# ArbiterMob/FluidSimulationCuda

Measured on AMD Instinct MI355X. Metric: Mcells/s per Jacobi iter, higher is better.
Workload: dtype f32

## Files before the change

### fluidsimulationcuda_amd/capi.py

```python
import ctypes as C
import os

import numpy as np

from ._build import LIB

OK, E_INVALID, E_NOMEM, E_HIP, E_COMM = 0, 1, 2, 3, 4
U, V, DENS, U_PREV, V_PREV, DENS_PREV, TMP0, TMP1, TMP2, TMP3, TMP4, TMP5 = range(12)
NFIELDS = 12
JACOBI_STREAM, JACOBI_LDS, JACOBI_NAIVE, JACOBI_TB = 0, 1, 2, 3
STORAGE_F32, STORAGE_F16 = 0, 1
PARAM_TB_MAX_SWEEPS, PARAM_TB_ROWS, PARAM_HALO, PARAM_TB_FAST_DIVISION, PARAM_TB_MIN_CELLS, PARAM_TB_EDGE_ROWS_PCT = 0, 1, 2, 3, 4, 5
PARAM_TB_LANE_COLUMNS = 6
PARAM_TB_T16_MIN_CELLS = 7
PARAM_TB_AUTOTUNE = 8
PARAM_FUSE_DIVERGENCE = 9
PARAM_SLAB_OVERLAP = 10
PARAM_EARLY_ADVECT = 11
PARAM_FUSE_ADD_SOURCE = 12
PARAM_XCHG_OVERLAP = 13
PARAM_F16_PRESSURE_SCALE = 14
PARAM_TB_FILL = 15
XCHG_HALO, XCHG_GATHER, XCHG_MAX, XCHG_MAX_BEGIN, XCHG_MAX_END = 0, 1, 2, 3, 4
RCCL_ID_BYTES = 128
FIELD_NAMES = ("u", "v", "dens", "u_prev", "v_prev", "dens_prev", "tmp0", "tmp1", "tmp2", "tmp3", "tmp4", "tmp5")


class FluidError(RuntimeError):
    def __init__(self, code, msg):
        super().__init__("libfluid_amd error %d: %s" % (code, msg))
        self.code = code


class Config(C.Structure):
    _fields_ = [("n", C.c_int), ("rank", C.c_int), ("nranks", C.c_int), ("halo", C.c_int),
                ("jacobi_variant", C.c_int), ("stream", C.c_void_p), ("arena", C.c_void_p),
                ("arena_bytes", C.c_size_t), ("storage", C.c_int)]
# ... 77 lines not shown
    "fluid_upload_members": [_ctx, _i, _MF],
    "fluid_run": [_ctx, _f, _f, _f, C.POINTER(RunPlan), C.POINTER(_i)],
    "fluid_run_members": [_ctx, _MF, _MF, _MF, C.POINTER(RunPlan), C.POINTER(_i)],
    "fluid_coarse_size": [_i, _i, C.POINTER(_i)],
    "fluid_pack_members_coarse": [_ctx, _i, _i, _i, _i, C.c_void_p, C.c_size_t],
    "fluid_download_members_coarse": [_ctx, _i, _i, _MF],
    "fluid_run_coarse": [_ctx, _f, _f, _f, C.POINTER(RunPlan), _i, C.POINTER(_i)],
    "fluid_run_members_coarse": [_ctx, _MF, _MF, _MF, C.POINTER(RunPlan), _i, C.POINTER(_i)],
    "fluid_transform_members": [_ctx, C.POINTER(_i), _i, _MF],
    "fluid_select_members": [_ctx, C.POINTER(_i), _i, C.POINTER(_i)],
    "fluid_set_jacobi_variant": [_ctx, _i],
    "fluid_division_mode": [_ctx, _f, _f, C.POINTER(_i)],
    "fluid_autotune_pending": [_ctx, C.POINTER(_i)],
    "fluid_plan_sweeps": [_i, _i, _i, _i, _i, _i, _i, C.POINTER(_i), _i, C.POINTER(_i)],
    "fluid_set_param": [_ctx, _i, _i],
    "fluid_timing_enable": [_ctx, _i],
    "fluid_timing_read": [_ctx, C.POINTER(Timing), _i],
    "fluid_op_diffuse_tol": [_ctx, _i, _i, _i, _f, _f, _f, _i, _i, C.POINTER(_i), C.POINTER(_f)],
    "fluid_set_exchange": [_ctx, EXCHANGE_FN, C.c_void_p],
    "fluid_exchange_now": [_ctx, _i, C.POINTER(_i), _i, _i],
    "fluid_exchange_stream": [_ctx, C.POINTER(C.c_void_p)],
    "fluid_split_launches": [_ctx, C.POINTER(C.c_longlong)],
    "fluid_rccl_available": [],
    "fluid_rccl_unique_id": [C.c_void_p, C.c_size_t],
    "fluid_exchange_rccl_attach": [_ctx, C.c_void_p, C.c_size_t],
    "fluid_exchange_rccl_attach_comm": [_ctx, C.c_void_p],
    "fluid_exchange_rccl_detach": [_ctx],
    "fluid_exchange_rccl_calls": [_ctx, C.POINTER(C.c_longlong), C.POINTER(C.c_longlong), C.POINTER(C.c_longlong)],
}
OTHER_SYMBOLS = {"fluid_last_error": (C.c_char_p, []), "fluid_arena_bytes": (C.c_size_t, [_i]),
# ... 34 lines not shown
```

### fluidsimulationcuda_amd/csrc/fluid_ctx.h

```cpp
#pragma once
#include <hip/hip_runtime.h>

#include <string>
#include <utility>
#include <vector>

#include "../../include/fluid_amd.h"
#include "fluid_kernels.h"

namespace fluid_detail {
int fail(int code, const char* fmt, ...);
int materialize_zero(fluid_ctx* c, int f);
int refuse_ensemble(const fluid_ctx* c, const char* what);
struct RcclExchange;
void rccl_release(RcclExchange* x);
}

#define HIP_TRY(expr)                                                                                      \
    do {                                                                                                   \
        hipError_t e_ = (expr);                                                                            \
        if (e_ != hipSuccess)                                                                              \
            return fluid_detail::fail(e_ == hipErrorOutOfMemory ? FLUID_E_NOMEM : FLUID_E_HIP, "%s: %s",   \
                                      #expr, hipGetErrorString(e_));                                       \
    } while (0)
// ... 88 lines not shown
    hipEvent_t ev_xbegin = nullptr, ev_xdone = nullptr;
    bool xchg_overlap = true;
    unsigned xowed = 0;
    long long split_launches = 0;
    bool early_advect = true;
    float vmax_prev[2] = {-1.0f, -1.0f};
    FieldState field[FLUID_NFIELDS];
    size_t field_bytes = 0;
    unsigned int* d_scalar = nullptr;
    float* d_partials = nullptr;
    ConstRing consts;
    EnsembleReduce red;
    MemberStage stage;
    TransformTables xform;
    unsigned int* tiles = nullptr;
    unsigned int* h_scalar = nullptr;
    hipEvent_t scalar_ready = nullptr;
    int variant = fluid::JACOBI_TB;
    int tb_max_t = 16, tb_rows = 0, num_cu = 256;
    long long tb_min_cells = 0;
    long long tb_t16_min_cells = -1;
    bool fuse_divergence = true;
    bool tb_fill = true;
    bool autotune = true;
    struct Trial { unsigned long long key; int cand; hipEvent_t a, b; };
    std::vector<Trial> trials;
    std::vector<hipEvent_t> free_events;
    bool defer_zero_source = true;
    bool in_halo_exchange = false;
    int tb_nv = 2;
// ... 29 lines not shown
```

### fluidsimulationcuda_amd/csrc/fluid_kernels.h

```cpp
#pragma once
#include <hip/hip_runtime.h>

namespace fluid {

constexpr int XOFF = 63;

enum JacobiVariant { JACOBI_STREAM = 0, JACOBI_LDS = 1, JACOBI_NAIVE = 2, JACOBI_TB = 3, JACOBI_VARIANTS = 4 };

enum Storage { STORAGE_F32 = 0, STORAGE_F16 = 1 };
typedef _Float16 half_t;
inline size_t storage_bytes(int st) { return st == STORAGE_F16 ? 2 : 4; }

inline int pitch_for(int n) { return ((XOFF + 1 + 4 * ((n + 3) / 4) + 1) + 63) / 64 * 64; }

struct Members {
    int count = 1;
    size_t stride = 0;
};

struct TbMemberK {
    double yd;
    float alpha, beta, hi, lo;
    float x0_inc, div_scale;
    unsigned tile_thr, pad;
};

struct TbBatch {
    const void* x[3];
    const void* x0[3];
    void* out[3];
    float alpha[3], beta[3];
    double yd[3];
    float hi[3], lo[3];
    const unsigned* tiles[3];
    unsigned tile_thr[3];
    int tile_pitch;
    void* div[3];
    float div_scale;
    int b[3];
    int x_zero[3];
    float x0_inc[3];
    int count;
    int members;
    size_t mstride;
    size_t tile_mstride;
    const TbMemberK* mk;
};

void launch_set_bnd(hipStream_t s, int st, void* f, int pitch, int n, int b, Members mb = {});
void launch_add_source(hipStream_t s, int st, void* x, const void* src, int pitch, int row_lo, int row_hi, float dt, Members mb = {},
                       const float* mdt = nullptr);
void launch_jacobi(hipStream_t s, int st, int variant, const void* x, const void* x0, void* out, int pitch, int n,
                   int row_lo, int row_hi, float alpha, float beta, int b, Members mb = {}, const float2* mab = nullptr);
enum TbForm { TB_PLAIN = 0, TB_DIVSRC = 1, TB_ADDSRC = 2 };
struct TbShape { int T, divmode, nv, form; };
inline constexpr TbShape kTbShapes[] = {
    {2, 0, 2, TB_PLAIN},   {2, 2, 2, TB_PLAIN},   {2, 3, 2, TB_PLAIN},   {2, 4, 2, TB_PLAIN},   {2, 5, 2, TB_PLAIN},
    {2, 0, 4, TB_PLAIN},   {2, 2, 4, TB_PLAIN},   {2, 3, 4, TB_PLAIN},   {2, 4, 4, TB_PLAIN},   {2, 5, 4, TB_PLAIN},
    {4, 0, 2, TB_PLAIN},   {4, 2, 2, TB_PLAIN},   {4, 3, 2, TB_PLAIN},   {4, 4, 2, TB_PLAIN},   {4, 5, 2, TB_PLAIN},
    {4, 0, 4, TB_PLAIN},   {4, 2, 4, TB_PLAIN},   {4, 3, 4, TB_PLAIN},   {4, 4, 4, TB_PLAIN},   {4, 5, 4, TB_PLAIN},
    {8, 0, 2, TB_PLAIN},   {8, 2, 2, TB_PLAIN},   {8, 3, 2, TB_PLAIN},   {8, 4, 2, TB_PLAIN},   {8, 5, 2, TB_PLAIN},
    {8, 0, 4, TB_PLAIN},   {8, 2, 4, TB_PLAIN},   {8, 3, 4, TB_PLAIN},   {8, 4, 4, TB_PLAIN},   {8, 5, 4, TB_PLAIN},
// ... 20 lines not shown
inline constexpr int kTbDepths[] = {16, 12, 8, 4, 2};
constexpr bool is_tb_depth(int T) { for (int d : kTbDepths) if (d == T) return true; return false; }
bool launch_jacobi_tb(hipStream_t s, int st, int T, int divmode, int nv, int form, const TbBatch& batch, int pitch, int n, int row_lo,
                      int row_hi, int rb, int rb_edge, int hole_lo = 0, int hole_hi = 0, bool fill = true);
constexpr int kTileRows = 32, kTileCols = 64;
inline int tile_rows(int n) { return (n + kTileRows - 1) / kTileRows; }
inline int tile_pitch(int n) { return (n + kTileCols - 1) / kTileCols; }
struct TileBatch {
    const void* field[3];
    unsigned* tiles[3];
    int count;
    size_t mstride, tile_mstride;
};
void launch_tile_min_abs(hipStream_t s, int st, const TileBatch& tb, int count, int pitch, int n, int row_lo, int row_hi, int tile_pitch,
                         Members mb = {}, size_t tile_mstride = 0);
void launch_validate_div(hipStream_t s, int divmode, float beta, float kbeta, double yd, float hi, float lo, unsigned long long* bad);
void launch_advect(hipStream_t s, int st, void* d, const void* d0, const void* u, const void* v, int pitch, int n,
                   int row_lo, int row_hi, float dt0, int b, Members mb = {}, const float* mdt0 = nullptr);
void launch_advect2(hipStream_t s, int st, void* da, const void* d0a, int ba, void* db, const void* d0b, int bb, const void* u,
                    const void* v, int pitch, int n, int row_lo, int row_hi, float dt0, Members mb = {}, const float* mdt0 = nullptr);
void launch_divergence(hipStream_t s, int st, const void* u, const void* v, void* p, void* div, int pitch, int n,
                       int row_lo, int row_hi, float h, int write_p, float pscale = 1.0f, Members mb = {});
void launch_scale(hipStream_t s, int st, void* x, int pitch, int row_lo, int row_hi, float factor, Members mb = {});
constexpr int kMaxPartials = 8192;
void launch_subtract_gradient(hipStream_t s, int st, void* u, void* v, const void* p, int pitch, int n, int row_lo,
                              int row_hi, float h, float* partials = nullptr, unsigned int* max_out = nullptr, float pinv = 1.0f,
                              Members mb = {});
void launch_gradient_advect(hipStream_t s, int st, void* u, void* v, const void* p, void* d, const void* d0, int pitch, int n,
                            int row_lo, int row_hi, float h, float dt0, int b, float pinv = 1.0f, Members mb = {},
                            const float* mdt0 = nullptr);
// ... 28 lines not shown
```

### fluidsimulationcuda_amd/csrc/fluid_kernels.hip

```cpp
#include <hip/hip_runtime.h>
#include <stdint.h>

#include <algorithm>
#include <array>
#include <cstdlib>
#include <utility>

#include "fluid_kernels.h"

namespace fluid {

__device__ __forceinline__ float flip_if(bool c, float v) { return c ? -v : v; }

__device__ __forceinline__ float keep_f32(float v) { asm("" : "+v"(v)); return v; }
__device__ __forceinline__ float ld1(const float* p) { return *p; }
__device__ __forceinline__ float ld1(const half_t* p) { return keep_f32((float)*p); }
__device__ __forceinline__ void st1(float* p, float v) { *p = v; }
__device__ __forceinline__ void st1(half_t* p, float v) { *p = (half_t)keep_f32(v); }
template <typename S>
__device__ __forceinline__ float as_stored(float v)
{
    if constexpr (sizeof(S) == 2) return keep_f32((float)(S)keep_f32(v));
    else return v;
}
// ... 781 lines not shown
        vid -= (unsigned)g.inner_blocks;
        const int e = (int)(vid % (unsigned)g.edge_wins);
        strip_group = (int)(vid / (unsigned)g.edge_wins);
        win = e == 0 ? 0 : g.first_right + e - 1;
    }
    const unsigned member = batch.count == 3 ? blockIdx.z / 3u : batch.count == 2 ? blockIdx.z >> 1 : blockIdx.z;
    const unsigned sv = blockIdx.z - member * (unsigned)batch.count;
    const size_t mofs = (size_t)member * batch.mstride;
    const S* __restrict__ x = static_cast<const S*>(batch.x[sv]) + mofs;
    const S* __restrict__ x0 = static_cast<const S*>(batch.x0[sv]) + mofs;
    S* __restrict__ out = static_cast<S*>(batch.out[sv]) + mofs;
    float alpha = batch.alpha[sv], beta = batch.beta[sv];
    double yd = batch.yd[sv];
    float k_hi = batch.hi[sv], k_lo = batch.lo[sv], x0_inc = batch.x0_inc[sv], div_scale = batch.div_scale;
    unsigned tile_thr = batch.tile_thr[sv];
    if (batch.mk != nullptr) {
        typedef const TbMemberK __attribute__((address_space(4))) * MemberKPtr;
        const MemberKPtr mk = (MemberKPtr)(uintptr_t)batch.mk + ((size_t)sv * (unsigned)batch.members + member);
        alpha = mk->alpha;
        beta = mk->beta;
        yd = mk->yd;
        k_hi = mk->hi;
        k_lo = mk->lo;
        x0_inc = mk->x0_inc;
        if (ADDSRC) div_scale = mk->div_scale;
        if (DIVMODE == 3) tile_thr = mk->tile_thr;
    }
    const int b = batch.b[sv];
    constexpr int HL = (T + NV - 1) / NV;
    constexpr int VS = 64 - 2 * HL;
    constexpr int C0 = (XOFF + 1) / NV;
    static_assert((XOFF + 1) % NV == 0 && HL <= C0, "window overlap must fit the row's left pad");
    const int lane = threadIdx.x & 63;
    const int strip = strip_group * 4 + __builtin_amdgcn_readfirstlane(threadIdx.x >> 6);
    const int kg = n / NV;
    const bool left_edge = (win == 0);
    const bool right_edge = (kg >= win * VS - HL) && (kg < win * VS - HL + 64);
    const bool edge = left_edge || right_edge;
    const int rbw = edge ? rb_edge : rb;
    TbArgs<S, NV> a;
    a.k.yd = yd;
// ... 37 lines not shown
    const bool is_rg = (k == kg);
    const bool own = (lane >= HL) && (lane < 64 - HL);
    const bool st_int = own && k >= 0 && k < nvec;
    a.st_rg_lane = is_rg && (own || k == nvec);
    a.m_lg = a.is_lg ? 0xFFFFFFFFu : 0u;
#pragma unroll
    for (int c = 0; c < NV; ++c) a.m_r[c] = (is_rg && a.cg == c) ? 0xFFFFFFFFu : 0u;
    a.st_off = (ld_ok && (st_int || a.is_lg || a.st_rg_lane)) ? a.ld_off : kBufOff;
    a.sx = (b == 1) ? 0x80000000u : 0u;
    a.sy = (b == 2) ? 0x80000000u : 0u;
    a.alpha = alpha;
    a.k.beta = beta;
    a.fill = fill != 0;
    const int t0 = max(0, a.q_lo - T), t1 = a.q_hi - 1 + T;
    const bool wall = (a.q_lo < T) || (a.q_hi - 1 + T > n + 1);
    constexpr int DM = DIVMODE == 3 ? 2 : DIVMODE;
    bool two_term = false;
    if constexpr (DIVMODE == 3) {
        const unsigned* __restrict__ tiles = batch.tiles[sv] ? batch.tiles[sv] + (size_t)member * batch.tile_mstride : nullptr;
        const unsigned thr = tile_thr;
        const int tr0 = (max(1, a.q_lo - T + 1) - 1) / kTileRows, tr1 = (min(n, a.q_hi + T - 2) - 1) / kTileRows;
        const int c0 = max(1, 1 + NV * (win * VS - HL)), c1 = min(n, NV * (win * VS - HL + 64));
        const int tc0 = (c0 - 1) / kTileCols, tc1 = (c1 - 1) / kTileCols, ntc = tc1 - tc0 + 1;
        const int count = (tr1 - tr0 + 1) * ntc;
        bool low = false;
        if (tiles != nullptr)
            for (int i = lane; i < count; i += 64)
                low |= tiles[(size_t)(tr0 + i / ntc) * batch.tile_pitch + (tc0 + i % ntc)] < thr;
        two_term = tiles != nullptr && __builtin_amdgcn_ballot_w64(low) == 0ull;
    }
// ... 19 lines not shown
    const int i0 = max(row_lo, 1 + tr * kTileRows), i1 = min(row_hi, 1 + (tr + 1) * kTileRows);
    const size_t P = (size_t)pitch;
    float m = __builtin_inff();
    if (j <= n)
        for (int i = i0; i < i1; ++i) {
            const float4 v = ld4(f + (size_t)i * P + XOFF + j);
            m = fminf(m, fabsf(v.x));
            if (j + 1 <= n) m = fminf(m, fabsf(v.y));
            if (j + 2 <= n) m = fminf(m, fabsf(v.z));
            if (j + 3 <= n) m = fminf(m, fabsf(v.w));
        }
#pragma unroll
    for (int off = 8; off > 0; off >>= 1) m = fminf(m, __shfl_xor(m, off, 16));
    const bool whole = row_lo <= 1 + tr * kTileRows && row_hi >= min(n + 1, 1 + (tr + 1) * kTileRows);
    if ((lane & 15) == 0 && j <= n) out[(size_t)tr * tile_pitch + (j - 1) / kTileCols] = whole ? __float_as_uint(m) : 0u;
}

template <typename S, typename IDX>
__device__ __forceinline__ const S* at(const S* base, IDX byte_off) { return reinterpret_cast<const S*>(reinterpret_cast<const char*>(base) + byte_off); }
template <typename S, typename IDX>
__device__ __forceinline__ S* at(S* base, IDX byte_off) { return reinterpret_cast<S*>(reinterpret_cast<char*>(base) + byte_off); }

template <typename IDX>
struct AdvectTap {
    IDX o;
    float s0, s1, t0, t1;
};

template <typename IDX>
__device__ __forceinline__ AdvectTap<IDX> advect_trace(int j, int i, float uu, float vv, float dt0, int n, IDX P, IDX E)
// ... 949 lines not shown
void launch_tile_min_abs(hipStream_t s, int st, const TileBatch& tiles, int count, int pitch, int n, int row_lo, int row_hi, int tile_pitch,
                         Members mb, size_t tile_mstride)
{
    if (row_lo < 1) row_lo = 1;
    if (row_hi > n + 1) row_hi = n + 1;
    if (row_hi <= row_lo || count <= 0) return;
    const int tr0 = (row_lo - 1) / kTileRows, tr1 = (row_hi - 2) / kTileRows;
    const dim3 grid(cdiv(cdiv(n, 4), 256), tr1 - tr0 + 1, count * mb.count);
    TileBatch tb = tiles;
    tb.count = count;
    tb.mstride = mb.stride;
    tb.tile_mstride = tile_mstride;
    FLUID_BY_STORAGE(st, hipLaunchKernelGGL(k_tile_min_abs<S>, grid, dim3(256), 0, s, tb, pitch, n, row_lo, row_hi, tr0, tile_pitch));
}

void launch_validate_div(hipStream_t s, int divmode, float beta, float kbeta, double yd, float hi, float lo, unsigned long long* bad)
{
    DivK k;
    k.beta = kbeta;
    k.yd = yd;
    k.hi = hi;
    k.lo = lo;
    const auto f = divmode == 4 ? k_validate_div<4> : divmode == 5 ? k_validate_div<5> : divmode == 3 ? k_validate_div<3> : k_validate_div<2>;
    hipLaunchKernelGGL(f, dim3(8192), dim3(256), 0, s, beta, k, bad);
}

void launch_advect(hipStream_t s, int st, void* d, const void* d0, const void* u, const void* v, int pitch, int n,
                   int row_lo, int row_hi, float dt0, int b, Members mb, const float* mdt0)
{
    if (row_hi <= row_lo) return;
// ... 199 lines not shown
```

### fluidsimulationcuda_amd/csrc/fluid_solver.hip

```cpp
#include <hip/hip_runtime.h>

#include <algorithm>
#include <cmath>
#include <cstdarg>
#include <cstdio>
#include <cstring>
#include <functional>
#include <mutex>
#include <new>
#include <string>
#include <unordered_map>
#include <vector>

#include "fluid_ctx.h"

namespace fluid_detail {

thread_local std::string g_err;

int fail(int code, const char* fmt, ...)
{
    char buf[512];
    va_list ap;
    va_start(ap, fmt);
// ... 638 lines not shown
                pickd = depth[k];
        if (!pickd) break;
        if (pickd <= room) best = std::max(best, pickd);
        r -= pickd;
    }
    return best ? best : greedy;
}

struct Coeffs {
    MemberVal alpha, beta;
};

struct Solve {
    int b, x, x0;
    const Coeffs* k;
};

struct DivSource {
    int u, v;
    float scale;
};

struct Batch {
    const Solve* sv;
    int count, iters, final_reach;
    const DivSource* ds;
    int scratch_base;
    const int* scratch;
    const int* sum;
    int cur[3], nxt[3];
    std::vector<DivPlan> plan[3];
    bool same_mode, all_mode4, add_src;
    float out_scale[3];
    SweepShape shape;
};

size_t tile_words(const fluid_ctx* c) { return (size_t)fluid::tile_rows(c->n) * fluid::tile_pitch(c->n); }
unsigned* solve_tiles(const fluid_ctx* c, int slot) { return c->tiles + (size_t)slot * c->members * tile_words(c); }

void plan_members(fluid_ctx* c, const Coeffs& k, std::vector<DivPlan>& out)
{
    const int M = c->members;
    const MemberVal &alpha = k.alpha, &beta = k.beta;
    out.resize(M);
    bool same = true;
    for (int m = 0; m < M; ++m) {
        out[m] = (m > 0 && beta.at(m) == beta.at(m - 1) && alpha.at(m) == alpha.at(m - 1)) ? out[m - 1] : division_mode(c, beta.at(m), alpha.at(m));
// ... 76 lines not shown
    }
    B.shape = sweep_shape(c, B.count);
    const FieldState& x00 = c->field[sv[0].x0];
    bool add_src = x00.src_of != 0 && B.ds == nullptr && B.same_mode;
    for (int k = 0; k < B.count; ++k) {
        const FieldState &x = c->field[sv[k].x], &x0 = c->field[sv[k].x0];
        add_src = add_src && x0.src_of == 1 + sv[k].x && x0.src_dt == x00.src_dt && !x.zero && !x.pend && !x.src_of;
    }
    B.add_src = add_src && fluid::jacobi_tb_exists(pick_sweeps(c, B.iters, B.iters, B.shape, B.all_mode4), B.plan[0][0].mode, c->tb_nv, fluid::TB_ADDSRC);
    if (!B.add_src)
        for (int k = 0; k < B.count; ++k)
            if (c->field[sv[k].x0].src_of) {
                TRY(xchg_join(c));
                TRY(settle_source(c, sv[k].x0));
            }
    fluid::TileBatch tb{};
    int m = 0, valid = kEverywhere;
    for (int k = 0; k < B.count; ++k)
        if (B.plan[k][0].mode == 3) {
            tb.field[m] = c->ptr(sv[k].x0);
            tb.tiles[m] = solve_tiles(c, B.scratch_base + k);
            valid = std::min(valid, c->nranks > 1 ? c->field[sv[k].x0].reach : kEverywhere);
            ++m;
        }
    if (m == 0) return FLUID_OK;
    TRY(xchg_join(c));
    if (c->nranks > 1)
        HIP_TRY(hipMemsetAsync(solve_tiles(c, B.scratch_base), 0, (size_t)B.count * c->members * tile_words(c) * sizeof(unsigned), c->stream));
    int lo, hi;
    rows(c, std::min(valid, c->n), &lo, &hi);
    fluid::launch_tile_min_abs(c->stream, c->st, tb, m, c->pitch, c->n, lo, hi, fluid::tile_pitch(c->n), c->mb(), tile_words(c));
    return FLUID_OK;
}

int batch_reach(const fluid_ctx* c, const Batch& B)
{
    int r = kEverywhere;
    for (int k = 0; k < B.count; ++k) r = std::min(r, std::min(c->field[B.cur[k]].reach, c->field[B.sv[k].x0].reach + 1));
    return r;
}

fluid::TbMemberK solve_constants(const Batch& B, int j, int m, const MemberVal& x0_inc, const MemberVal& div_scale)
{
    const DivPlan& p = B.plan[j][B.plan[j].size() > 1 ? (size_t)m : 0];
    return {p.yd, B.sv[j].k->alpha.at(m), p.arg, p.hi, p.lo, x0_inc.at(m), div_scale.at(m), p.tile_thr, 0};
}

int fill_batch(fluid_ctx* c, const Batch& B, int first, int last, bool divsrc, bool addsrc, fluid::TbBatch* out)
{
    static const MemberVal nothing_pending(-0.0f);
    const MemberVal own_scale(divsrc ? B.ds->scale : 0.0f);
    const MemberVal& div_scale = addsrc ? c->field[B.sv[first].x0].src_dt : own_scale;
    const MemberVal* x0_inc[3];
    fluid::TbBatch bt{};
    bool per_member = !div_scale.uniform();
    for (int j = first; j < last; ++j) {
        const int q = j - first;
        const FieldState& x0 = c->field[B.sv[j].x0];
        x0_inc[q] = x0.pend && !addsrc && !divsrc ? &x0.pend_inc : &nothing_pending;
        per_member = per_member || B.plan[j].size() > 1 || !x0_inc[q]->uniform();
        const fluid::TbMemberK k0 = solve_constants(B, j, 0, *x0_inc[q], div_scale);
        bt.x[q] = c->ptr(B.cur[j]);
        bt.x0[q] = x0.ptr;
        bt.out[q] = c->ptr(B.nxt[j]);
        bt.alpha[q] = k0.alpha;
        bt.beta[q] = k0.beta;
        bt.yd[q] = k0.yd;
        bt.hi[q] = k0.hi;
        bt.lo[q] = k0.lo;
        bt.tiles[q] = B.plan[j][0].mode == 3 ? solve_tiles(c, B.scratch_base + j) : nullptr;
        bt.tile_thr[q] = k0.tile_thr;
        bt.b[q] = B.sv[j].b;
        bt.x_zero[q] = c->field[B.cur[j]].zero ? 1 : 0;
        bt.x0_inc[q] = k0.x0_inc;
        if (addsrc) bt.div[q] = c->ptr(B.sum[j]);
    }
    bt.count = last - first;
    bt.members = c->members;
    bt.mstride = c->field_floats;
    bt.tile_mstride = tile_words(c);
    bt.tile_pitch = fluid::tile_pitch(c->n);
    bt.div_scale = div_scale.at(0);
    if (divsrc) {
        bt.x[0] = c->ptr(B.ds->u);
        bt.x0[0] = c->ptr(B.ds->v);
        bt.div[0] = c->ptr(B.sv[0].x0);
    }
    if (per_member && c->members > 1) {
        const int M = c->members;
        std::vector<fluid::TbMemberK> rec((size_t)bt.count * M);
        for (int j = first; j < last; ++j)
            for (int m = 0; m < M; ++m) rec[(size_t)(j - first) * M + m] = solve_constants(B, j, m, *x0_inc[j - first], div_scale);
        const void* dev = nullptr;
        TRY(member_consts(c, rec.data(), rec.size() * sizeof rec[0], &dev));
        bt.mk = static_cast<const fluid::TbMemberK*>(dev);
    }
    *out = bt;
    return FLUID_OK;
}

int edge_rows(const fluid_ctx* c, int T, int rb) { return std::max(2 * T, rb * (c->tb_edge_pct > 0 ? c->tb_edge_pct : 100) / 100); }

int strip_rows(const fluid_ctx* c, int T, int m, long long rows_n)
{
    const int nv = c->tb_nv;
    const int HL = (T + nv - 1) / nv, VS = 64 - 2 * HL;
    const long long windows = ((c->n + nv - 1) / nv + VS - 1) / VS;
// ... 99 lines not shown
            for (int j = 0; j < B.count; ++j) {
                const float2* mab = nullptr;
                TRY(member_pairs(c, sv[j].k->alpha, sv[j].k->beta, &mab));
                fluid::launch_jacobi(c->stream, c->st, v, c->ptr(B.cur[j]), c->ptr(sv[j].x0), c->ptr(B.nxt[j]), c->pitch, c->n, lo, hi,
                                     sv[j].k->alpha.at(0), sv[j].k->beta.at(0), sv[j].b, c->mb(), mab);
            }
            if (c->timing) {
                c->launches += B.count;
                c->field_launches += (long long)B.count * c->members;
            }
        } else {
            for (int first = 0, last; first < B.count; first = last) {
                last = B.same_mode ? B.count : first + 1;
                const bool divsrc = B.ds != nullptr && k == 0, addsrc = B.add_src && k == 0;
                fluid::TbBatch bt;
                TRY(fill_batch(c, B, first, last, divsrc, addsrc, &bt));
                TRY(launch_fused(c, bt, T, B.plan[first][0].mode, divsrc, addsrc, lo, hi));
                if (c->timing) {
                    c->launches += 1;
                    c->field_launches += (long long)(last - first) * c->members;
                }
            }
        }
        r = multi ? std::min(r - T, exchange_cap(c)) : kEverywhere;
        commit_launch(c, B, k == 0, r);
        k += T;
    }
    return FLUID_OK;
}

int op_diffuse_batch(fluid_ctx* c, const Solve* sv, int count, int iters, int final_reach = 0, const DivSource* ds = nullptr,
// ... 241 lines not shown
    const Solve uv[2] = {{1, U0, U, &cv}, {2, V0, V, &cv}};
    TRY(op_diffuse_batch(c, uv, 2, iters));
    TRY(xchg_join(c));
    TRY(project(c, U0, V0, U, V, iters, nullptr, true));
    const float dt0 = dt.at(0) * (float)c->n;
    TRY(vmax_begin(c, U0, V0, true));
    TRY(advect_bounded(c, 0, {U0, V0}, dt0, [&] { return op_advect2(c, 1, U, U0, 2, V, V0, U0, V0, dt); }));
    return project(c, U, V, U0, V0, iters);
}

int dens_step(fluid_ctx* c, const MemberVal& dt, const MemberVal& diff, int iters)
{
    const int X = FLUID_DENS, X0 = FLUID_DENS_PREV;
    TRY(op_add_source(c, X, X0, dt, true));
    const Coeffs cd = diffusion_coeffs(c, dt, diff);
    const Solve one{0, X0, X, &cd};
    TRY(op_diffuse_batch(c, &one, 1, iters));
    TRY(vmax_begin(c, FLUID_U, FLUID_V));
    return advect_bounded(c, 1, {X0}, dt.at(0) * (float)c->n, [&] { return op_advect(c, 0, X, X0, FLUID_U, FLUID_V, dt); });
}

int full_step(fluid_ctx* c, const MemberVal& dt, const MemberVal& diff, const MemberVal& visc, int iters)
{
    const int U = FLUID_U, V = FLUID_V, D = FLUID_DENS, U0 = FLUID_U_PREV, V0 = FLUID_V_PREV, D0 = FLUID_DENS_PREV;
    TRY(op_add_source(c, U, U0, dt, true));
    TRY(op_add_source(c, V, V0, dt, true));
    TRY(op_add_source(c, D, D0, dt, true));
    TRY(need(c, {U, V, D, U0, V0, D0}, std::min(iters, c->halo), true));
    const Coeffs cv = diffusion_coeffs(c, dt, visc), cd = diffusion_coeffs(c, dt, diff);
    const float dt0 = dt.at(0) * (float)c->n;
    const Solve all[3] = {{1, U0, U, &cv}, {2, V0, V, &cv}, {0, D0, D, &cd}};
    if (c->nranks == 1) {
        TRY(op_diffuse_batch(c, all, 3, iters));
        TRY(project(c, U0, V0, U, V, iters));
        TRY(op_advect2(c, 1, U, U0, 2, V, V0, U0, V0, dt));
        const AdvectAfter dens{0, D, D0, dt};
        return project(c, U, V, U0, V0, iters, &dens);
    }
    int fill1 = 0, fill2 = 0;
    {
        const SweepShape shape = sweep_shape(c, 1);
        std::vector<int> launches;
        for (int left = iters; left > 0;) {
            launches.push_back(pick_sweeps(c, left, left, shape, false));
            left -= launches.back();
        }
        for (int* fill : {&fill2, &fill1})
            while (*fill < 8 && !launches.empty()) {
// ... 203 lines not shown
    if (P > 1) {
        if (!hip_ok(hipStreamCreateWithFlags(&c->stream2, hipStreamNonBlocking), "hipStreamCreate(second stream)")) return bail(rc);
        if (!hip_ok(hipEventCreateWithFlags(&c->ev_fork, hipEventDisableTiming), "hipEventCreate")) return bail(rc);
        if (!hip_ok(hipEventCreateWithFlags(&c->ev_join, hipEventDisableTiming), "hipEventCreate")) return bail(rc);
        if (!hip_ok(hipStreamCreateWithFlags(&c->xstream, hipStreamNonBlocking), "hipStreamCreate(exchange stream)")) return bail(rc);
        if (!hip_ok(hipEventCreateWithFlags(&c->ev_xbegin, hipEventDisableTiming), "hipEventCreate")) return bail(rc);
        if (!hip_ok(hipEventCreateWithFlags(&c->ev_xdone, hipEventDisableTiming), "hipEventCreate")) return bail(rc);
    }
    if (!hip_ok(hipMemsetAsync(c->arena, 0, bytes, c->stream), "hipMemsetAsync(arena)")) return bail(rc);
    c->d_scalar = reinterpret_cast<unsigned int*>(c->arena + c->all_bytes() * FLUID_NFIELDS);
    {
        const size_t words = 3 * (size_t)members * tile_words(c);
        if (!hip_ok(hipMalloc((void**)&c->tiles, words * sizeof(unsigned)), "hipMalloc(tiles)")) return bail(rc);
        if (!hip_ok(hipMemsetAsync(c->tiles, 0, words * sizeof(unsigned), c->stream), "hipMemsetAsync(tiles)")) return bail(rc);
    }
    if (P > 1 && !hip_ok(hipMalloc((void**)&c->d_partials, fluid::kMaxPartials * sizeof(float)), "hipMalloc(partials)")) return bail(rc);
    if (!hip_ok(hipHostMalloc((void**)&c->h_scalar, 256, hipHostMallocDefault), "hipHostMalloc")) return bail(rc);
    if (!hip_ok(hipEventCreateWithFlags(&c->scalar_ready, hipEventDisableTiming), "hipEventCreate")) return bail(rc);
    if (!hip_ok(hipStreamSynchronize(c->stream), "hipStreamSynchronize")) return bail(rc);
    *out = c;
    return FLUID_OK;
}

int fluid_create(int N, fluid_ctx** out)
{
    fluid_config cfg;
    std::memset(&cfg, 0, sizeof cfg);
    cfg.n = N;
    cfg.nranks = 1;
    cfg.jacobi_variant = FLUID_JACOBI_TB;
// ... 13 lines not shown
    if (!c->trials.empty()) {
        RbTuner& t = rb_tuner();
        std::lock_guard<std::mutex> lock(t.mu);
        for (auto& tr : c->trials) {
            auto it = t.table.find(tr.key);
            if (it != t.table.end() && !it->second.fixed && it->second.issued[tr.cand] > 0) it->second.issued[tr.cand] -= 1;
            (void)hipEventDestroy(tr.a);
            (void)hipEventDestroy(tr.b);
        }
    }
    for (hipEvent_t ev : c->free_events) (void)hipEventDestroy(ev);
    fluid_detail::rccl_release(c->rccl);
    c->rccl = nullptr;
    if (c->h_scalar) (void)hipHostFree(c->h_scalar);
    if (c->tiles) (void)hipFree(c->tiles);
    for (auto& b : c->consts.live) (void)hipEventDestroy(b.copied);
    for (hipEvent_t ev : c->consts.free_events) (void)hipEventDestroy(ev);
    if (c->consts.dev) (void)hipFree(c->consts.dev);
    if (c->consts.host) (void)hipHostFree(c->consts.host);
    if (c->red.d_max) (void)hipFree(c->red.d_max);
    if (c->red.d_moments) (void)hipFree(c->red.d_moments);
    if (c->red.d_partials) (void)hipFree(c->red.d_partials);
    if (c->red.host) (void)hipHostFree(c->red.host);
    if (c->red.d_mean) (void)hipFree(c->red.d_mean);
    if (c->red.d_var) (void)hipFree(c->red.d_var);
    if (c->red.d_gram_partials) (void)hipFree(c->red.d_gram_partials);
    if (c->red.d_gram) (void)hipFree(c->red.d_gram);
    if (c->red.gram_host) (void)hipHostFree(c->red.gram_host);
    if (c->stage.dev) (void)hipFree(c->stage.dev);
    for (hipEvent_t ev : c->xform.copied)
// ... 23 lines not shown
}

int fluid_exchange_stream(fluid_ctx* c, void** stream)
{
    TRY(check_ctx(c));
    if (!stream) return fail(FLUID_E_INVALID, "null pointer");
    *stream = c->stream;
    return FLUID_OK;
}

int fluid_split_launches(fluid_ctx* c, long long* count)
{
    TRY(check_ctx(c));
    if (!count) return fail(FLUID_E_INVALID, "null pointer");
    *count = c->split_launches;
    return FLUID_OK;
}

int fluid_owned_rows(fluid_ctx* c, int* row_lo, int* row_hi)
{
    TRY(check_ctx(c));
    if (row_lo) *row_lo = c->own0;
    if (row_hi) *row_hi = c->own1;
    return FLUID_OK;
}

int fluid_field_ptr(fluid_ctx* c, int field, void** dev_ptr)
{
    TRY(check_ctx(c));
    TRY(check_fields(c, {field}));
// ... 155 lines not shown
        c->pscale = (value != 0 && c->st == fluid::STORAGE_F16 && c->n >= 16) ? std::ldexp(1.0f, e - 3) : 1.0f;
        return FLUID_OK;
    }
    case FLUID_PARAM_XCHG_OVERLAP:
        TRY(xchg_join(c));
        c->xchg_overlap = value != 0;
        return FLUID_OK;
    case FLUID_PARAM_TB_T16_MIN_CELLS:
        if (value < -1) return fail(FLUID_E_INVALID, "TB_T16_MIN_CELLS must be >= 0, or -1 for the default rule");
        c->tb_t16_min_cells = value;
        return FLUID_OK;
    case FLUID_PARAM_TB_LANE_COLUMNS:
        if (value != 2 && value != 4) return fail(FLUID_E_INVALID, "TB_LANE_COLUMNS must be 2 or 4");
        c->tb_nv = value;
        return FLUID_OK;
    case FLUID_PARAM_HALO:
        if (value < 1) return fail(FLUID_E_INVALID, "HALO must be >= 1");
        c->halo = c->nranks > 1 ? std::max(c->st == fluid::STORAGE_F16 ? 8 : 1, std::min(value, c->min_slab - 1)) : 1;
        return FLUID_OK;
    default:
        return fail(FLUID_E_INVALID, "unknown parameter %d", key);
    }
}

int fluid_plan_sweeps(int N, int rows, int storage, int pressure_form, int iters, int max_sweeps, int t16_min_cells, int* depths,
                      int capacity, int* count)
{
    if (N < 1 || N > kMaxN || rows < 1 || rows > N || iters < 0 || (iters & 1) || !depths || !count || capacity < 0)
        return fail(FLUID_E_INVALID, "fluid_plan_sweeps: bad argument");
    if (storage != FLUID_STORAGE_F32 && storage != FLUID_STORAGE_F16) return fail(FLUID_E_INVALID, "unknown storage type %d", storage);
// ... 1011 lines not shown
```

### fluidsimulationcuda_amd/solver.py

```python
import ctypes as C
import sys

import numpy as np

from . import capi

DT, VIS, DIFF, ITERS = 0.016, 0.0025, 0.1, 40

_ID = {name: k for k, name in enumerate(capi.FIELD_NAMES)}


def _fid(f):
    if isinstance(f, str):
        return _ID[f]
    return int(f)


def _host(a, n):
    a = np.ascontiguousarray(a, dtype=np.float32)
    if a.shape != (n + 2, n + 2):
        raise ValueError("field must have shape (%d, %d), got %s" % (n + 2, n + 2, a.shape))
    return a


# ... 321 lines not shown
            out[name + "_ms"] = t.category_ms[k]
            out[name + "_calls"] = t.category_calls[k]
        return out

    def diffuse_tol(self, b, x, x0, alpha, beta, tol, max_iters=10000, check_every=8):
        it, res = C.c_int(), C.c_float()
        capi.check(capi.lib().fluid_op_diffuse_tol(self._h, b, _fid(x), _fid(x0), alpha, beta, tol, max_iters,
                                                   check_every, C.byref(it), C.byref(res)))
        return it.value, res.value

    def split_launches(self):
        m = C.c_longlong()
        capi.check(capi.lib().fluid_split_launches(self._h, C.byref(m)))
        return m.value

    def exchange_stream(self):
        p = C.c_void_p()
        capi.check(capi.lib().fluid_exchange_stream(self._h, C.byref(p)))
        return p.value or 0

    def set_exchange(self, fn):
        if fn is None:
            self._cb = None
            capi.check(capi.lib().fluid_set_exchange(self._h, C.cast(None, capi.EXCHANGE_FN), None))
            return

        def tramp(_user, kind, fields, nfields, depth, scalar):
            try:
                ids = [fields[k] for k in range(nfields)]
                if kind in (capi.XCHG_MAX, capi.XCHG_MAX_END):
# ... 38 lines not shown
```

### include/fluid_amd.h

```cpp
#ifndef FLUID_AMD_H
#define FLUID_AMD_H

#include <stddef.h>

#ifdef __cplusplus
extern "C" {
#endif

#define FLUID_OK        0
#define FLUID_E_INVALID 1
#define FLUID_E_NOMEM   2
#define FLUID_E_HIP     3
#define FLUID_E_COMM    4

enum {
    FLUID_U = 0, FLUID_V = 1, FLUID_DENS = 2,
    FLUID_U_PREV = 3, FLUID_V_PREV = 4, FLUID_DENS_PREV = 5,
    FLUID_TMP0 = 6, FLUID_TMP1 = 7, FLUID_TMP2 = 8,
    FLUID_TMP3 = 9, FLUID_TMP4 = 10, FLUID_TMP5 = 11,
    FLUID_NFIELDS = 12
};

enum { FLUID_JACOBI_STREAM = 0, FLUID_JACOBI_LDS = 1, FLUID_JACOBI_NAIVE = 2, FLUID_JACOBI_TB = 3 };

// ... 1 lines not shown
    FLUID_PARAM_TB_MAX_SWEEPS = 0,
    FLUID_PARAM_TB_ROWS = 1,
    FLUID_PARAM_HALO = 2,
    FLUID_PARAM_TB_FAST_DIVISION = 3
    ,FLUID_PARAM_TB_EDGE_ROWS_PCT = 5
    ,FLUID_PARAM_TB_LANE_COLUMNS = 6
    ,FLUID_PARAM_TB_T16_MIN_CELLS = 7
    ,FLUID_PARAM_TB_AUTOTUNE = 8
    ,FLUID_PARAM_SLAB_OVERLAP = 10
    ,FLUID_PARAM_EARLY_ADVECT = 11
    ,FLUID_PARAM_FUSE_DIVERGENCE = 9
    ,FLUID_PARAM_FUSE_ADD_SOURCE = 12
    ,FLUID_PARAM_XCHG_OVERLAP = 13
    ,FLUID_PARAM_F16_PRESSURE_SCALE = 14
    ,FLUID_PARAM_TB_FILL = 15
    ,FLUID_PARAM_TB_MIN_CELLS = 4
};

typedef struct fluid_ctx fluid_ctx;

const char *fluid_last_error(void);

int step(int N, float dt, float diff, float visc, float *u, float *v, float *dens);
int step_src(int N, float dt, float diff, float visc, int iters,
             float *u, float *v, float *dens,
             float *u_prev, float *v_prev, float *dens_prev);
int fluid_release_cached(void);

int fluid_coefficients(int N, float dt, float coef, float *alpha, float *beta);

// ... 93 lines not shown
int fluid_run_coarse(fluid_ctx *ctx, float dt, float diff, float visc, const fluid_run_plan *plan, int factor,
                     int *snapshots_written);
int fluid_run_members_coarse(fluid_ctx *ctx, const float *dt, const float *diff, const float *visc,
                             const fluid_run_plan *plan, int factor, int *snapshots_written);

#define FLUID_TRANSFORM_MAX_MEMBERS 64
int fluid_transform_members(fluid_ctx *ctx, const int *fields, int nfields, const float *weights);
int fluid_select_members(fluid_ctx *ctx, const int *fields, int nfields, const int *source);

int fluid_set_jacobi_variant(fluid_ctx *ctx, int variant);
int fluid_division_mode(fluid_ctx *ctx, float alpha, float beta, int *mode);
int fluid_plan_sweeps(int N, int rows, int storage, int pressure_form, int iters, int max_sweeps, int t16_min_cells,
                      int *depths, int capacity, int *count);
int fluid_autotune_pending(fluid_ctx *ctx, int *shapes_open);
int fluid_set_param(fluid_ctx *ctx, int key, int value);

enum {
    FLUID_TIME_SOURCE = 0, FLUID_TIME_DIFFUSION = 1, FLUID_TIME_DIVERGENCE = 2,
    FLUID_TIME_PROJECTION = 3, FLUID_TIME_ADVECTION = 4, FLUID_TIMING_CATEGORIES = 5
};
typedef struct fluid_timing {
    double jacobi_ms;
    long long sweeps;
    long long solves;
    double category_ms[FLUID_TIMING_CATEGORIES];
    long long category_calls[FLUID_TIMING_CATEGORIES];
    long long jacobi_launches;
    long long jacobi_field_launches;
    double pressure_ms;
    long long pressure_sweeps;
// ... 30 lines not shown
```

Measured before the change: 4.278 million.

## Skip Jacobi work on all-zero density tiles via per-tile nonzero bitmaps

Adds a pre-pass kernel that ORs the bit patterns of the density right-hand side and initial guess into a per-tile map. The temporally blocked Jacobi kernel checks, per wavefront, whether every tile inside its dependency cone (widened by the sweep index) is zero, and if so writes zeros and returns instead of computing. Density is reordered to be first in the batched diffusion solve, and device-side atomic counters record how many waves skip. The change adds a map-building pass and atomics on every launch, and it only pays off when the density field is sparse.

```diff
diff --git a/fluidsimulationcuda_amd/capi.py b/fluidsimulationcuda_amd/capi.py
--- a/fluidsimulationcuda_amd/capi.py
+++ b/fluidsimulationcuda_amd/capi.py
@@ -21,6 +21,7 @@
 PARAM_XCHG_OVERLAP = 13
 PARAM_F16_PRESSURE_SCALE = 14
 PARAM_TB_FILL = 15
+PARAM_SPARSE_DENSITY = 16
 XCHG_HALO, XCHG_GATHER, XCHG_MAX, XCHG_MAX_BEGIN, XCHG_MAX_END = 0, 1, 2, 3, 4
 RCCL_ID_BYTES = 128
 FIELD_NAMES = ("u", "v", "dens", "u_prev", "v_prev", "dens_prev", "tmp0", "tmp1", "tmp2", "tmp3", "tmp4", "tmp5")
@@ -128,6 +129,7 @@
     "fluid_autotune_pending": [_ctx, C.POINTER(_i)],
     "fluid_plan_sweeps": [_i, _i, _i, _i, _i, _i, _i, C.POINTER(_i), _i, C.POINTER(_i)],
     "fluid_set_param": [_ctx, _i, _i],
+    "fluid_sparse_stats": [_ctx, C.POINTER(C.c_ulonglong)],
     "fluid_timing_enable": [_ctx, _i],
     "fluid_timing_read": [_ctx, C.POINTER(Timing), _i],
     "fluid_op_diffuse_tol": [_ctx, _i, _i, _i, _f, _f, _f, _i, _i, C.POINTER(_i), C.POINTER(_f)],
diff --git a/fluidsimulationcuda_amd/csrc/fluid_ctx.h b/fluidsimulationcuda_amd/csrc/fluid_ctx.h
--- a/fluidsimulationcuda_amd/csrc/fluid_ctx.h
+++ b/fluidsimulationcuda_amd/csrc/fluid_ctx.h
@@ -126,6 +126,8 @@
     MemberStage stage;
     TransformTables xform;
     unsigned int* tiles = nullptr;
+    bool sparse_density = true;
+    unsigned long long* d_zstats = nullptr;
     unsigned int* h_scalar = nullptr;
     hipEvent_t scalar_ready = nullptr;
     int variant = fluid::JACOBI_TB;
diff --git a/fluidsimulationcuda_amd/csrc/fluid_kernels.h b/fluidsimulationcuda_amd/csrc/fluid_kernels.h
--- a/fluidsimulationcuda_amd/csrc/fluid_kernels.h
+++ b/fluidsimulationcuda_amd/csrc/fluid_kernels.h
@@ -22,7 +22,8 @@
     double yd;
     float alpha, beta, hi, lo;
     float x0_inc, div_scale;
-    unsigned tile_thr, pad;
+    unsigned tile_thr;
+    unsigned sparse;
 };
 
 struct TbBatch {
@@ -45,7 +46,12 @@
     size_t mstride;
     size_t tile_mstride;
     const TbMemberK* mk;
+    const unsigned* zmap[3];
+    int zmap_k0;
+    unsigned long long* zstats;
 };
+constexpr int kSparseStatSlots = 64, kSparseStatStride = 16;
+constexpr size_t kSparseStatWords = (size_t)kSparseStatSlots * kSparseStatStride;
 
 void launch_set_bnd(hipStream_t s, int st, void* f, int pitch, int n, int b, Members mb = {});
 void launch_add_source(hipStream_t s, int st, void* x, const void* src, int pitch, int row_lo, int row_hi, float dt, Members mb = {},
@@ -96,6 +102,8 @@
 };
 void launch_tile_min_abs(hipStream_t s, int st, const TileBatch& tb, int count, int pitch, int n, int row_lo, int row_hi, int tile_pitch,
                          Members mb = {}, size_t tile_mstride = 0);
+void launch_tile_or_bits(hipStream_t s, int st, const void* rhs, const void* guess, unsigned* map, int pitch, int n, int tile_pitch,
+                         Members mb = {}, size_t tile_mstride = 0);
 void launch_validate_div(hipStream_t s, int divmode, float beta, float kbeta, double yd, float hi, float lo, unsigned long long* bad);
 void launch_advect(hipStream_t s, int st, void* d, const void* d0, const void* u, const void* v, int pitch, int n,
                    int row_lo, int row_hi, float dt0, int b, Members mb = {}, const float* mdt0 = nullptr);
diff --git a/fluidsimulationcuda_amd/csrc/fluid_kernels.hip b/fluidsimulationcuda_amd/csrc/fluid_kernels.hip
--- a/fluidsimulationcuda_amd/csrc/fluid_kernels.hip
+++ b/fluidsimulationcuda_amd/csrc/fluid_kernels.hip
@@ -819,6 +819,8 @@
     double yd = batch.yd[sv];
     float k_hi = batch.hi[sv], k_lo = batch.lo[sv], x0_inc = batch.x0_inc[sv], div_scale = batch.div_scale;
     unsigned tile_thr = batch.tile_thr[sv];
+    constexpr bool CAN_SKIP = !DIVSRC && DIVMODE != 4;
+    bool sparse = CAN_SKIP && batch.zmap[sv] != nullptr;
     if (batch.mk != nullptr) {
         typedef const TbMemberK __attribute__((address_space(4))) * MemberKPtr;
         const MemberKPtr mk = (MemberKPtr)(uintptr_t)batch.mk + ((size_t)sv * (unsigned)batch.members + member);
@@ -830,6 +832,7 @@
         x0_inc = mk->x0_inc;
         if (ADDSRC) div_scale = mk->div_scale;
         if (DIVMODE == 3) tile_thr = mk->tile_thr;
+        if (CAN_SKIP && sparse) sparse = mk->sparse != 0u;
     }
     const int b = batch.b[sv];
     constexpr int HL = (T + NV - 1) / NV;
@@ -897,6 +900,34 @@
     a.fill = fill != 0;
     const int t0 = max(0, a.q_lo - T), t1 = a.q_hi - 1 + T;
     const bool wall = (a.q_lo < T) || (a.q_hi - 1 + T > n + 1);
+    if constexpr (CAN_SKIP) {
+        if (sparse && !edge && !wall) {
+            const unsigned* __restrict__ zm = batch.zmap[sv] + (size_t)member * batch.tile_mstride;
+            const int k0 = batch.zmap_k0;
+            const int tr0 = (max(1, a.q_lo - T - k0) - 1) / kTileRows, tr1 = (min(n, a.q_hi - 1 + T + k0) - 1) / kTileRows;
+            const int c0 = max(1, 1 + NV * (win * VS - HL) - k0), c1 = min(n, NV * (win * VS - HL + 64) + k0);
+            const int tc0 = (c0 - 1) / kTileCols, tc1 = (c1 - 1) / kTileCols, ntc = tc1 - tc0 + 1;
+            const int count = (tr1 - tr0 + 1) * ntc;
+            bool nz = false;
+            for (int i = lane; i < count; i += 64) nz |= zm[(size_t)(tr0 + i / ntc) * batch.tile_pitch + (tc0 + i % ntc)] != 0u;
+            const bool skip = __builtin_amdgcn_ballot_w64(nz) == 0ull;
+            if (lane == 0) {
+                unsigned long long* slot = batch.zstats + (blockIdx.x % kSparseStatSlots) * (size_t)kSparseStatStride;
+                atomicAdd(slot + 1, 1ull);
+                if (skip) atomicAdd(slot, 1ull);
+            }
+            if (skip) {
+                Vec<NV> zero;
+#pragma unroll
+                for (int c = 0; c < NV; ++c) zero.c[c] = 0.f;
+                for (int q = a.q_lo; q < a.q_hi; ++q) {
+                    buf_stv<NV>(a.oc, a.bo, a.st_off + (unsigned)q * a.row_bytes, zero);
+                    if constexpr (ADDSRC) buf_stv<NV>(a.dc, a.bd, a.st_off + (unsigned)q * a.row_bytes, zero);
+                }
+                return;
+            }
+        }
+    }
     constexpr int DM = DIVMODE == 3 ? 2 : DIVMODE;
     bool two_term = false;
     if constexpr (DIVMODE == 3) {
@@ -946,6 +977,43 @@
     for (int off = 8; off > 0; off >>= 1) m = fminf(m, __shfl_xor(m, off, 16));
     const bool whole = row_lo <= 1 + tr * kTileRows && row_hi >= min(n + 1, 1 + (tr + 1) * kTileRows);
     if ((lane & 15) == 0 && j <= n) out[(size_t)tr * tile_pitch + (j - 1) / kTileCols] = whole ? __float_as_uint(m) : 0u;
+}
+
+template <typename S>
+__global__ __launch_bounds__(256) void k_tile_or_bits(const S* __restrict__ rhs, const S* __restrict__ guess, unsigned* __restrict__ map,
+                                                      int pitch, int n, int tile_pitch, size_t mstride, size_t tile_mstride)
+{
+    const unsigned member = blockIdx.z;
+    rhs += (size_t)member * mstride;
+    if (guess != nullptr) guess += (size_t)member * mstride;
+    unsigned* __restrict__ out = map + (size_t)member * tile_mstride;
+    const int lane = threadIdx.x & 63, wave = threadIdx.x >> 6;
+    const int tr = blockIdx.y;
+    const int j = 1 + 4 * (lane + 64 * (blockIdx.x * 4 + wave));
+    const int i0 = 1 + tr * kTileRows, i1 = min(n + 1, i0 + kTileRows);
+    const size_t P = (size_t)pitch;
+    const unsigned m1 = j + 1 <= n ? ~0u : 0u, m2 = j + 2 <= n ? ~0u : 0u, m3 = j + 3 <= n ? ~0u : 0u;
+    auto row_bits = [&](const S* f, int i) {
+        const float4 v = ld4(f + (size_t)i * P + XOFF + j);
+        return __float_as_uint(v.x) | (__float_as_uint(v.y) & m1) | (__float_as_uint(v.z) & m2) | (__float_as_uint(v.w) & m3);
+    };
+    unsigned bits = 0u;
+    if (j <= n) {
+        if (guess == nullptr) {
+            for (int i = i0; i < i1; ++i) bits |= row_bits(rhs, i);
+        } else {
+            for (int i = i0; i < i1; ++i) bits |= row_bits(rhs, i) | row_bits(guess, i);
+            if (i0 == 1) bits |= row_bits(guess, 0);
+            if (i1 == n + 1) bits |= row_bits(guess, n + 1);
+            if (j == 1)
+                for (int i = i0; i < i1; ++i) bits |= __float_as_uint(ld1(guess + (size_t)i * P + XOFF));
+            if (j + 3 >= n)
+                for (int i = i0; i < i1; ++i) bits |= __float_as_uint(ld1(guess + (size_t)i * P + XOFF + n + 1));
+        }
+    }
+#pragma unroll
+    for (int off = 8; off > 0; off >>= 1) bits |= (unsigned)__shfl_xor((int)bits, off, 16);
+    if ((lane & 15) == 0 && j <= n) out[(size_t)tr * tile_pitch + (j - 1) / kTileCols] = bits;
 }
 
 template <typename S, typename IDX>
@@ -1925,6 +1993,14 @@
     FLUID_BY_STORAGE(st, hipLaunchKernelGGL(k_tile_min_abs<S>, grid, dim3(256), 0, s, tb, pitch, n, row_lo, row_hi, tr0, tile_pitch));
 }
 
+void launch_tile_or_bits(hipStream_t s, int st, const void* rhs, const void* guess, unsigned* map, int pitch, int n, int tile_pitch,
+                         Members mb, size_t tile_mstride)
+{
+    const dim3 grid(cdiv(cdiv(n, 4), 256), tile_rows(n), mb.count);
+    FLUID_BY_STORAGE(st, hipLaunchKernelGGL(k_tile_or_bits<S>, grid, dim3(256), 0, s, (const S*)rhs, (const S*)guess, map, pitch, n,
+                                            tile_pitch, mb.stride, tile_mstride));
+}
+
 void launch_validate_div(hipStream_t s, int divmode, float beta, float kbeta, double yd, float hi, float lo, unsigned long long* bad)
 {
     DivK k;
diff --git a/fluidsimulationcuda_amd/csrc/fluid_solver.hip b/fluidsimulationcuda_amd/csrc/fluid_solver.hip
--- a/fluidsimulationcuda_amd/csrc/fluid_solver.hip
+++ b/fluidsimulationcuda_amd/csrc/fluid_solver.hip
@@ -676,6 +676,7 @@
 struct Solve {
     int b, x, x0;
     const Coeffs* k;
+    bool sparse = false;
 };
 
 struct DivSource {
@@ -693,6 +694,7 @@
     int cur[3], nxt[3];
     std::vector<DivPlan> plan[3];
     bool same_mode, all_mode4, add_src;
+    bool zmap[3];
     float out_scale[3];
     SweepShape shape;
 };
@@ -799,6 +801,14 @@
                 TRY(xchg_join(c));
                 TRY(settle_source(c, sv[k].x0));
             }
+    for (int k = 0; k < B.count; ++k) {
+        B.zmap[k] = sv[k].sparse && c->sparse_density && c->nranks == 1 && B.ds == nullptr && B.plan[k][0].mode != 3 &&
+                    B.plan[k][0].mode != 4 && pick_sweeps(c, B.iters, B.iters, B.shape, B.all_mode4) > 1;
+        if (!B.zmap[k]) continue;
+        const FieldState& x = c->field[sv[k].x];
+        fluid::launch_tile_or_bits(c->stream, c->st, c->ptr(sv[k].x0), x.zero ? nullptr : x.ptr, solve_tiles(c, B.scratch_base + k),
+                                   c->pitch, c->n, fluid::tile_pitch(c->n), c->mb(), tile_words(c));
+    }
     fluid::TileBatch tb{};
     int m = 0, valid = kEverywhere;
     for (int k = 0; k < B.count; ++k)
@@ -825,13 +835,16 @@
     return r;
 }
 
-fluid::TbMemberK solve_constants(const Batch& B, int j, int m, const MemberVal& x0_inc, const MemberVal& div_scale)
+fluid::TbMemberK solve_constants(const Batch& B, int j, int m, const MemberVal& x0_inc, const MemberVal& div_scale, bool addsrc)
 {
     const DivPlan& p = B.plan[j][B.plan[j].size() > 1 ? (size_t)m : 0];
-    return {p.yd, B.sv[j].k->alpha.at(m), p.arg, p.hi, p.lo, x0_inc.at(m), div_scale.at(m), p.tile_thr, 0};
-}
-
-int fill_batch(fluid_ctx* c, const Batch& B, int first, int last, bool divsrc, bool addsrc, fluid::TbBatch* out)
+    const float alpha = B.sv[j].k->alpha.at(m), beta = B.sv[j].k->beta.at(m);
+    const bool sparse = B.zmap[j] && std::isfinite(alpha) && std::isfinite(beta) && beta > 0.0f && x0_inc.at(m) == 0.0f &&
+                        (!addsrc || std::isfinite(div_scale.at(m)));
+    return {p.yd, alpha, p.arg, p.hi, p.lo, x0_inc.at(m), div_scale.at(m), p.tile_thr, sparse ? 1u : 0u};
+}
+
+int fill_batch(fluid_ctx* c, const Batch& B, int first, int last, bool divsrc, bool addsrc, int k0, fluid::TbBatch* out)
 {
     static const MemberVal nothing_pending(-0.0f);
     const MemberVal own_scale(divsrc ? B.ds->scale : 0.0f);
@@ -844,22 +857,25 @@
         const FieldState& x0 = c->field[B.sv[j].x0];
         x0_inc[q] = x0.pend && !addsrc && !divsrc ? &x0.pend_inc : &nothing_pending;
         per_member = per_member || B.plan[j].size() > 1 || !x0_inc[q]->uniform();
-        const fluid::TbMemberK k0 = solve_constants(B, j, 0, *x0_inc[q], div_scale);
+        const fluid::TbMemberK r0 = solve_constants(B, j, 0, *x0_inc[q], div_scale, addsrc);
         bt.x[q] = c->ptr(B.cur[j]);
         bt.x0[q] = x0.ptr;
         bt.out[q] = c->ptr(B.nxt[j]);
-        bt.alpha[q] = k0.alpha;
-        bt.beta[q] = k0.beta;
-        bt.yd[q] = k0.yd;
-        bt.hi[q] = k0.hi;
-        bt.lo[q] = k0.lo;
+        bt.alpha[q] = r0.alpha;
+        bt.beta[q] = r0.beta;
+        bt.yd[q] = r0.yd;
+        bt.hi[q] = r0.hi;
+        bt.lo[q] = r0.lo;
         bt.tiles[q] = B.plan[j][0].mode == 3 ? solve_tiles(c, B.scratch_base + j) : nullptr;
-        bt.tile_thr[q] = k0.tile_thr;
+        bt.tile_thr[q] = r0.tile_thr;
         bt.b[q] = B.sv[j].b;
         bt.x_zero[q] = c->field[B.cur[j]].zero ? 1 : 0;
-        bt.x0_inc[q] = k0.x0_inc;
+        bt.x0_inc[q] = r0.x0_inc;
         if (addsrc) bt.div[q] = c->ptr(B.sum[j]);
-    }
+        bt.zmap[q] = B.zmap[j] && !divsrc && r0.sparse ? solve_tiles(c, B.scratch_base + j) : nullptr;
+    }
+    bt.zmap_k0 = k0;
+    bt.zstats = c->d_zstats;
     bt.count = last - first;
     bt.members = c->members;
     bt.mstride = c->field_floats;
@@ -875,7 +891,10 @@
         const int M = c->members;
         std::vector<fluid::TbMemberK> rec((size_t)bt.count * M);
         for (int j = first; j < last; ++j)
-            for (int m = 0; m < M; ++m) rec[(size_t)(j - first) * M + m] = solve_constants(B, j, m, *x0_inc[j - first], div_scale);
+            for (int m = 0; m < M; ++m) {
+                rec[(size_t)(j - first) * M + m] = solve_constants(B, j, m, *x0_inc[j - first], div_scale, addsrc);
+                if (rec[(size_t)(j - first) * M + m].sparse && !divsrc) bt.zmap[j - first] = solve_tiles(c, B.scratch_base + j);
+            }
         const void* dev = nullptr;
         TRY(member_consts(c, rec.data(), rec.size() * sizeof rec[0], &dev));
         bt.mk = static_cast<const fluid::TbMemberK*>(dev);
@@ -1005,7 +1024,7 @@
                 last = B.same_mode ? B.count : first + 1;
                 const bool divsrc = B.ds != nullptr && k == 0, addsrc = B.add_src && k == 0;
                 fluid::TbBatch bt;
-                TRY(fill_batch(c, B, first, last, divsrc, addsrc, &bt));
+                TRY(fill_batch(c, B, first, last, divsrc, addsrc, k, &bt));
                 TRY(launch_fused(c, bt, T, B.plan[first][0].mode, divsrc, addsrc, lo, hi));
                 if (c->timing) {
                     c->launches += 1;
@@ -1277,7 +1296,7 @@
     const int X = FLUID_DENS, X0 = FLUID_DENS_PREV;
     TRY(op_add_source(c, X, X0, dt, true));
     const Coeffs cd = diffusion_coeffs(c, dt, diff);
-    const Solve one{0, X0, X, &cd};
+    const Solve one{0, X0, X, &cd, true};
     TRY(op_diffuse_batch(c, &one, 1, iters));
     TRY(vmax_begin(c, FLUID_U, FLUID_V));
     return advect_bounded(c, 1, {X0}, dt.at(0) * (float)c->n, [&] { return op_advect(c, 0, X, X0, FLUID_U, FLUID_V, dt); });
@@ -1292,9 +1311,10 @@
     TRY(need(c, {U, V, D, U0, V0, D0}, std::min(iters, c->halo), true));
     const Coeffs cv = diffusion_coeffs(c, dt, visc), cd = diffusion_coeffs(c, dt, diff);
     const float dt0 = dt.at(0) * (float)c->n;
-    const Solve all[3] = {{1, U0, U, &cv}, {2, V0, V, &cv}, {0, D0, D, &cd}};
+    const Solve all[3] = {{1, U0, U, &cv}, {2, V0, V, &cv}, {0, D0, D, &cd, true}};
     if (c->nranks == 1) {
-        TRY(op_diffuse_batch(c, all, 3, iters));
+        const Solve dens_first[3] = {all[2], all[0], all[1]};
+        TRY(op_diffuse_batch(c, dens_first, 3, iters));
         TRY(project(c, U0, V0, U, V, iters));
         TRY(op_advect2(c, 1, U, U0, 2, V, V0, U0, V0, dt));
         const AdvectAfter dens{0, D, D0, dt};
@@ -1528,6 +1548,8 @@
         if (!hip_ok(hipMalloc((void**)&c->tiles, words * sizeof(unsigned)), "hipMalloc(tiles)")) return bail(rc);
         if (!hip_ok(hipMemsetAsync(c->tiles, 0, words * sizeof(unsigned), c->stream), "hipMemsetAsync(tiles)")) return bail(rc);
     }
+    if (!hip_ok(hipMalloc((void**)&c->d_zstats, fluid::kSparseStatWords * sizeof(unsigned long long)), "hipMalloc(sparse stats)")) return bail(rc);
+    if (!hip_ok(hipMemsetAsync(c->d_zstats, 0, fluid::kSparseStatWords * sizeof(unsigned long long), c->stream), "hipMemsetAsync(sparse stats)")) return bail(rc);
     if (P > 1 && !hip_ok(hipMalloc((void**)&c->d_partials, fluid::kMaxPartials * sizeof(float)), "hipMalloc(partials)")) return bail(rc);
     if (!hip_ok(hipHostMalloc((void**)&c->h_scalar, 256, hipHostMallocDefault), "hipHostMalloc")) return bail(rc);
     if (!hip_ok(hipEventCreateWithFlags(&c->scalar_ready, hipEventDisableTiming), "hipEventCreate")) return bail(rc);
@@ -1571,6 +1593,7 @@
     c->rccl = nullptr;
     if (c->h_scalar) (void)hipHostFree(c->h_scalar);
     if (c->tiles) (void)hipFree(c->tiles);
+    if (c->d_zstats) (void)hipFree(c->d_zstats);
     for (auto& b : c->consts.live) (void)hipEventDestroy(b.copied);
     for (hipEvent_t ev : c->consts.free_events) (void)hipEventDestroy(ev);
     if (c->consts.dev) (void)hipFree(c->consts.dev);
@@ -1624,6 +1647,22 @@
     TRY(check_ctx(c));
     if (!count) return fail(FLUID_E_INVALID, "null pointer");
     *count = c->split_launches;
+    return FLUID_OK;
+}
+
+int fluid_sparse_stats(fluid_ctx* c, unsigned long long out[2])
+{
+    TRY(check_ctx(c));
+    if (!out) return fail(FLUID_E_INVALID, "null pointer");
+    std::vector<unsigned long long> slots(fluid::kSparseStatWords);
+    HIP_TRY(hipMemcpyAsync(slots.data(), c->d_zstats, slots.size() * sizeof slots[0], hipMemcpyDeviceToHost, c->stream));
+    HIP_TRY(hipMemsetAsync(c->d_zstats, 0, slots.size() * sizeof slots[0], c->stream));
+    HIP_TRY(hipStreamSynchronize(c->stream));
+    out[0] = out[1] = 0;
+    for (int s = 0; s < fluid::kSparseStatSlots; ++s) {
+        out[0] += slots[(size_t)s * fluid::kSparseStatStride];
+        out[1] += slots[(size_t)s * fluid::kSparseStatStride + 1];
+    }
     return FLUID_OK;
 }
 
@@ -1809,6 +1848,9 @@
         if (value != 2 && value != 4) return fail(FLUID_E_INVALID, "TB_LANE_COLUMNS must be 2 or 4");
         c->tb_nv = value;
         return FLUID_OK;
+    case FLUID_PARAM_SPARSE_DENSITY:
+        c->sparse_density = value != 0;
+        return FLUID_OK;
     case FLUID_PARAM_HALO:
         if (value < 1) return fail(FLUID_E_INVALID, "HALO must be >= 1");
         c->halo = c->nranks > 1 ? std::max(c->st == fluid::STORAGE_F16 ? 8 : 1, std::min(value, c->min_slab - 1)) : 1;
diff --git a/fluidsimulationcuda_amd/solver.py b/fluidsimulationcuda_amd/solver.py
--- a/fluidsimulationcuda_amd/solver.py
+++ b/fluidsimulationcuda_amd/solver.py
@@ -359,6 +359,11 @@
         capi.check(capi.lib().fluid_split_launches(self._h, C.byref(m)))
         return m.value
 
+    def sparse_stats(self):
+        out = (C.c_ulonglong * 2)()
+        capi.check(capi.lib().fluid_sparse_stats(self._h, out))
+        return int(out[0]), int(out[1])
+
     def exchange_stream(self):
         p = C.c_void_p()
         capi.check(capi.lib().fluid_exchange_stream(self._h, C.byref(p)))
diff --git a/include/fluid_amd.h b/include/fluid_amd.h
--- a/include/fluid_amd.h
+++ b/include/fluid_amd.h
@@ -39,6 +39,7 @@
     ,FLUID_PARAM_XCHG_OVERLAP = 13
     ,FLUID_PARAM_F16_PRESSURE_SCALE = 14
     ,FLUID_PARAM_TB_FILL = 15
+    ,FLUID_PARAM_SPARSE_DENSITY = 16
     ,FLUID_PARAM_TB_MIN_CELLS = 4
 };
 
@@ -162,6 +163,7 @@
                       int *depths, int capacity, int *count);
 int fluid_autotune_pending(fluid_ctx *ctx, int *shapes_open);
 int fluid_set_param(fluid_ctx *ctx, int key, int value);
+int fluid_sparse_stats(fluid_ctx *ctx, unsigned long long out[2]);
 
 enum {
     FLUID_TIME_SOURCE = 0, FLUID_TIME_DIFFUSION = 1, FLUID_TIME_DIVERGENCE = 2,
```

After: 4.302 million, median of 6. About the same (+0.6%).
